# neggles/neurosis

Measured on AMD Instinct MI355X. Metric: train images/sec (node) SDXL 1024^2, higher is better.
Workload: dtype bf16

## Files before the change

### neurosis_amd/csrc/gemm.hip

```cpp
#include "nk_common.h"
#include "nk_gemm.h"
#include <stdlib.h>

#define BM 128
#define BN 128
#define BK 64
#define NTHREADS 256
#define GROUP_M 8
#define KC_IMAGE_BYTES (128 * 128)
#define MC_ROW_BYTES (128 * 2 + 16)
#define MC_IMAGE_BYTES (BK * MC_ROW_BYTES)
#define OPND_BYTES MC_IMAGE_BYTES
#define STAGE_BYTES (2 * OPND_BYTES)
#define CS_LD 132
#define SMEM_BYTES (2 * STAGE_BYTES)

static_assert(SMEM_BYTES >= BM * CS_LD * 4, "epilogue staging must fit");

enum { OP_KC = 0, OP_KCG = 1, OP_MC = 2, OP_MCT = 3, OP_MCG = 4 };

__device__ __forceinline__ bool is_kc(int mode) { return mode == OP_KC || mode == OP_KCG; }

__device__ __forceinline__ long gather_offset(const NkGather& g, int n, int bh, int bw, int kh, int kw,
                                              int c, bool& valid) {
// ... 1097 lines not shown
            int spins = 0;
            bool gave_up = (p.sk_debug & 2) != 0;
            while (!gave_up && __hip_atomic_load(p.sk_flags + ticket, __ATOMIC_RELAXED, __HIP_MEMORY_SCOPE_AGENT) == 0u) {
              __builtin_amdgcn_s_sleep(8);
              if (++spins > (1 << 21)) gave_up = true;
            }
            if (gave_up) {
              if (tid == 0) {
                __hip_atomic_store(p.sk_flags + SK_MAX_GRID + 1, 1u, __ATOMIC_RELAXED, __HIP_MEMORY_SCOPE_AGENT);
                __hip_atomic_store(p.sk_health, 1u, __ATOMIC_RELAXED, __HIP_MEMORY_SCOPE_AGENT);
              }
              const float poison = __builtin_nanf("");
#pragma unroll
              for (int i = 0; i < 4; ++i)
#pragma unroll
                for (int j = 0; j < 2; ++j) acc[i][j] = (float4_t){poison, poison, poison, poison};
              break;
            }
            sk_add_partial(p.sk_ws + (size_t)ticket * SK_TILE_FLOATS, acc, wave, lane);
            __syncthreads();
            if (tid == 0) __hip_atomic_store(p.sk_flags + ticket, 0u, __ATOMIC_RELAXED, __HIP_MEMORY_SCOPE_AGENT);
          }
          if (s_li <= ts) break;
        }
      }
      sk_epilogue<OUT_F32>(p, C, acc, m0, n0, lane, wm, wn);
    }
  }
}

#define XL_BM 256
#define XL_BN 256
#define XL_STAGE_BYTES 65536
#define XL_SMEM_BYTES (2 * XL_STAGE_BYTES)
template <int AMODE, int WM, int WN>
__global__ __launch_bounds__((XL_BM / WM) * (XL_BN / WN) * 64, (XL_BM / WM) * (XL_BN / WN) / 4) void nk_gemm_xl_kernel(const NkGemmParams p) {
  extern __shared__ __attribute__((aligned(16))) char smem[];
  constexpr int WCOLS = XL_BN / WN, NWAVES = (XL_BM / WM) * WCOLS, NP = 32 / NWAVES, MI = WM / 16, NJ = WN / 16;
  const int tid = threadIdx.x, lane = tid & 63, wave = tid >> 6;
  const int wm = wave / WCOLS, wn = wave % WCOLS;
  const int nwg = gridDim.x, bid = blockIdx.x;
  const int q8 = nwg >> 3, r8 = nwg & 7, xcd = bid & 7;
  const int wg = (xcd < r8 ? xcd * (q8 + 1) : r8 * (q8 + 1) + (xcd - r8) * q8) + (bid >> 3);
  const int ntn = (p.N + XL_BN - 1) / XL_BN, ntm = (p.M + XL_BM - 1) / XL_BM;
  constexpr int GM = 4;
  const int per_group = GM * ntn;
  const int group = wg / per_group;
  const int first_m = group * GM;
  const int gm = min(GM, ntm - first_m);
  const int in_group = wg - group * per_group;
  const int nt = in_group / gm;
  const int m0 = (first_m + (in_group - nt * gm)) * XL_BM, n0 = nt * XL_BN;
  const int kend = p.K, nk = (p.K + BK - 1) / BK;

  OperandDMA<AMODE, NP> opa;
  OperandDMA<OP_KC, NP> opb;
  opa.init(p.A, p.lda, p.M, m0, tid, p.ga);
  opb.init(p.B, p.ldb, p.N, n0, tid, p.gb);
  float4_t acc[MI][NJ];
#pragma unroll
  for (int i = 0; i < MI; ++i)
#pragma unroll
    for (int j = 0; j < NJ; ++j) acc[i][j] = (float4_t){0.f, 0.f, 0.f, 0.f};
  opa.start(0);
  opb.start(0);
  if (nk > 0) {
    opa.issue_next(kend, smem, p.ga, p.tw);
    opb.issue_next(kend, smem + 32768, p.gb, p.tw);
  }
  for (int kt = 0; kt < nk; ++kt) {
    asm volatile("s_waitcnt vmcnt(0)" ::: "memory");
    __syncthreads();
    const char* cur = smem + (kt & 1) * XL_STAGE_BYTES;
    if (kt + 1 < nk) {
      char* nxt = smem + ((kt + 1) & 1) * XL_STAGE_BYTES;
      opa.issue_next(kend, nxt, p.ga, p.tw);
      opb.issue_next(kend, nxt + 32768, p.gb, p.tw);
    }
#pragma unroll
    for (int ks = 0; ks < 2; ++ks) {
      bf16x8_t af[MI], bfr[NJ];
#pragma unroll
      for (int i = 0; i < MI; ++i) af[i] = OperandDMA<OP_KC>::frag(cur, wm * WM + i * 16, ks, lane);
#pragma unroll
      for (int j = 0; j < NJ; ++j) bfr[j] = OperandDMA<OP_KC>::frag(cur + 32768, wn * WN + j * 16, ks, lane);
#pragma unroll
      for (int i = 0; i < MI; ++i)
#pragma unroll
        for (int j = 0; j < NJ; ++j)
          acc[i][j] = __builtin_amdgcn_mfma_f32_16x16x32_bf16(bfr[j], af[i], acc[i][j], 0, 0, 0);
    }
  }
#pragma unroll
  for (int ib = 0; ib < MI / 4; ++ib)
#pragma unroll
    for (int half = 0; half < NJ / 2; ++half) {
      float4_t pair[4][2];
#pragma unroll
      for (int i = 0; i < 4; ++i) { pair[i][0] = acc[ib * 4 + i][2 * half]; pair[i][1] = acc[ib * 4 + i][2 * half + 1]; }
      reg_epilogue_64x32<0>(p, p.C, pair, m0 + wm * WM + ib * 64, n0 + wn * WN + half * 32, lane);
    }
}

template <int AMODE, int GEGLU = 0>
__global__ __launch_bounds__(512, 2) void nk_gemm_xl2g_kernel(const NkGemmParams p) {
  extern __shared__ __attribute__((aligned(16))) char smem[];
  const int tid = threadIdx.x, lane = tid & 63, wave = tid >> 6;
  const int wm = wave >> 2, wn = wave & 3;
  const int nwg = gridDim.x, bid = blockIdx.x;
  const int q8 = nwg >> 3, r8 = nwg & 7, xcd = bid & 7;
  const int wg = (xcd < r8 ? xcd * (q8 + 1) : r8 * (q8 + 1) + (xcd - r8) * q8) + (bid >> 3);
  const int ntn = (p.N + XL_BN - 1) / XL_BN, ntm = (p.M + XL_BM - 1) / XL_BM;
  constexpr int GM = 4;
  const int per_group = GM * ntn;
  const int group = wg / per_group;
  const int first_m = group * GM;
  const int gm = min(GM, ntm - first_m);
  const int in_group = wg - group * per_group;
  const int nt = in_group / gm;
  const int m0 = (first_m + (in_group - nt * gm)) * XL_BM, n0 = nt * XL_BN;
  const int kend = p.K, nk = (p.K + BK - 1) / BK;

  OperandDMA<AMODE, 2> a0, a1;
  OperandDMA<OP_KC, 2> b0, b1;
  a0.init(p.A, p.lda, p.M, m0, tid, p.ga);
  a1.init(p.A, p.lda, p.M, m0 + 128, tid, p.ga);
  if constexpr (GEGLU) {
    const int I = p.N >> 1, wv = tid >> 6;
    const int gb0 = wv, gb1 = 8 + wv;
    b0.init(p.B, p.ldb, p.N, ((gb0 & 1) ? I : 0) + (n0 >> 1) + (gb0 >> 1) * 16 - wv * 16, tid, p.gb);
    b1.init(p.B, p.ldb, p.N, ((gb1 & 1) ? I : 0) + (n0 >> 1) + (gb1 >> 1) * 16 - wv * 16, tid, p.gb);
  } else {
    b0.init(p.B, p.ldb, p.N, n0, tid, p.gb);
    b1.init(p.B, p.ldb, p.N, n0 + 128, tid, p.gb);
  }
  const int s0 = p.k_rotate ? (xcd * nk) >> 3 : 0;
  const int wrap_at = nk - s0;
  int na0 = 0, na1 = 0, nb0 = 0, nb1 = 0, ka0 = kend, ka1 = kend, kb0 = kend, kb1 = kend;
  a0.start(s0 * BK); a1.start(s0 * BK); b0.start(s0 * BK); b1.start(s0 * BK);
#define X2_NEXT(op, src, g, cnt, ke)                        \
  do {                                                      \
    op.next_sources(ke, src, g, p.tw);                      \
    if (++cnt == wrap_at) { op.start(0); ke = s0 * BK; }    \
  } while (0)
#define X2_ISSUE(op, img, g, cnt, ke)                       \
  do {                                                      \
    const bf16_t* s_[2];                                    \
    X2_NEXT(op, s_, g, cnt, ke);                            \
    op.fire(0, s_[0], img); op.fire(1, s_[1], img);         \
  } while (0)
  float4_t acc[8][4];
#pragma unroll
  for (int i = 0; i < 8; ++i)
#pragma unroll
    for (int j = 0; j < 4; ++j) acc[i][j] = (float4_t){0.f, 0.f, 0.f, 0.f};

  bf16x8_t ar[8], bc0[4], bc1[4];
  typedef __attribute__((address_space(3))) const char* lds_c;
  const unsigned lds0 = (unsigned)(size_t)(lds_c)smem;
  const unsigned x0 = (unsigned)(((lane >> 4) ^ (lane & 7)) << 4);
  const unsigned arow = lds0 + (unsigned)(wm * 128 + (lane & 15)) * 128u;
  const unsigned brow = lds0 + 32768u + (unsigned)(wn * 64 + (lane & 15)) * 128u;
  const unsigned a_k0 = arow + x0, a_k1 = arow + (x0 ^ 64u), b_k0 = brow + x0, b_k1 = brow + (x0 ^ 64u);
#define X2_RD1(f, addr, OFF) asm volatile("ds_read_b128 %0, %1 offset:%2" : "=v"(f) : "v"(addr), "n"((OFF)))
#define X2_RDA(half)                                                                                             \
  X2_RD1(ar[0], ca0, (half) * 8192); X2_RD1(ar[1], ca0, (half) * 8192 + 2048); X2_RD1(ar[2], ca0, (half) * 8192 + 4096);    \
  X2_RD1(ar[3], ca0, (half) * 8192 + 6144); X2_RD1(ar[4], ca1, (half) * 8192); X2_RD1(ar[5], ca1, (half) * 8192 + 2048);    \
  X2_RD1(ar[6], ca1, (half) * 8192 + 4096); X2_RD1(ar[7], ca1, (half) * 8192 + 6144)
#define X2_RDB(f, half)                                                                                          \
  X2_RD1(f[0], cb0, (half) * 4096); X2_RD1(f[1], cb0, (half) * 4096 + 2048); X2_RD1(f[2], cb1, (half) * 4096);              \
  X2_RD1(f[3], cb1, (half) * 4096 + 2048)
#define X2_BAR() __builtin_amdgcn_sched_barrier(0); __builtin_amdgcn_s_barrier(); __builtin_amdgcn_sched_barrier(0)
#define X2_MM(rb, cb, bf, PREP)                                                                                  \
  asm volatile("s_waitcnt lgkmcnt(0)" ::: "memory");                                                             \
  __builtin_amdgcn_sched_barrier(0);                                                                             \
  __builtin_amdgcn_s_setprio(1);                                                                                 \
  PREP;               \
  _Pragma("unroll") for (int ks = 0; ks < 2; ++ks)                                                               \
    _Pragma("unroll") for (int i = 0; i < 4; ++i)                                                                \
      _Pragma("unroll") for (int j = 0; j < 2; ++j)                                                              \
        acc[(rb) + i][(cb) + j] = __builtin_amdgcn_mfma_f32_16x16x32_bf16(bf[ks * 2 + j], ar[ks * 4 + i], acc[(rb) + i][(cb) + j], 0, 0, 0); \
  __builtin_amdgcn_s_setprio(0)

  const bf16_t* sa0[2];
  const bf16_t* sa1[2];
  const bf16_t* sb0[2];
  const bf16_t* sb1[2];
  if (nk > 0) {
    X2_ISSUE(a0, smem, p.ga, na0, ka0);
    X2_ISSUE(a1, smem + 16384, p.ga, na1, ka1);
    X2_ISSUE(b0, smem + 32768, p.gb, nb0, kb0);
    X2_ISSUE(b1, smem + 49152, p.gb, nb1, kb1);
    X2_ISSUE(b0, smem + XL_STAGE_BYTES + 32768, p.gb, nb0, kb0);
    X2_ISSUE(b1, smem + XL_STAGE_BYTES + 49152, p.gb, nb1, kb1);
    asm volatile("s_waitcnt vmcnt(4)" ::: "memory");
  }
  X2_NEXT(a1, sa1, p.ga, na1, ka1);
  X2_BAR();
  if (wm == 1) { X2_BAR(); }
  for (int t = 0; t < nk; ++t) {
    const unsigned so = (unsigned)(t & 1) * XL_STAGE_BYTES;
    char* cur = smem + so;
    char* oth = smem + (so ^ XL_STAGE_BYTES);
    const unsigned ca0 = a_k0 + so, ca1 = a_k1 + so, cb0 = b_k0 + so, cb1 = b_k1 + so;
    __builtin_amdgcn_sched_barrier(0);
    X2_RDB(bc0, 0);
    X2_RDA(0);
    a1.fire(0, sa1[0], oth + 16384);
    a1.fire(1, sa1[1], oth + 16384);
    X2_BAR();
    X2_MM(0, 0, bc0, X2_NEXT(a0, sa0, p.ga, na0, ka0));
    X2_BAR();
    X2_RDB(bc1, 1);
    a0.fire(0, sa0[0], oth);
    a0.fire(1, sa0[1], oth);
    X2_BAR();
    X2_MM(0, 2, bc1, (void)0);
    X2_BAR();
    X2_RDA(1);
    X2_BAR();
    X2_MM(4, 2, bc1, X2_NEXT(b0, sb0, p.gb, nb0, kb0); X2_NEXT(b1, sb1, p.gb, nb1, kb1));
    X2_BAR();
    b0.fire(0, sb0[0], cur + 32768);
    b0.fire(1, sb0[1], cur + 32768);
    b1.fire(0, sb1[0], cur + 49152);
    b1.fire(1, sb1[1], cur + 49152);
    asm volatile("s_waitcnt vmcnt(4)" ::: "memory");
    X2_BAR();
    X2_MM(4, 0, bc0, X2_NEXT(a1, sa1, p.ga, na1, ka1));
    X2_BAR();
  }
  if (wm == 0) { X2_BAR(); }
  asm volatile("s_waitcnt vmcnt(0)" ::: "memory");
#undef X2_NEXT
#undef X2_ISSUE
#undef X2_RD1
#undef X2_RDA
#undef X2_RDB
#undef X2_BAR
#undef X2_MM
  if constexpr (GEGLU) {
    const int I = p.N >> 1;
    const int abase = (n0 >> 1) + wn * 32;
    const int cl = (lane >> 4) * 4;
    float4_t ba[2], bg[2];
#pragma unroll
    for (int q = 0; q < 2; ++q) {
      ba[q] = p.bias ? *(const float4_t*)(p.bias + abase + q * 16 + cl) : (float4_t){0.f, 0.f, 0.f, 0.f};
      bg[q] = p.bias ? *(const float4_t*)(p.bias + I + abase + q * 16 + cl) : (float4_t){0.f, 0.f, 0.f, 0.f};
    }
    NkGemmParams ph = p;
    ph.N = I; ph.ldc = p.ld_h; ph.bias = nullptr;
    NkGemmParams ps = p;
    ps.bias = nullptr;
#pragma unroll
    for (int ib = 0; ib < 2; ++ib) {
      float4_t pa[4][2], pg[4][2], phh[4][2];
#pragma unroll
      for (int i = 0; i < 4; ++i)
#pragma unroll
        for (int q = 0; q < 2; ++q) {
          pa[i][q] = acc[ib * 4 + i][2 * q];
          pg[i][q] = acc[ib * 4 + i][2 * q + 1];
#pragma unroll
          for (int r = 0; r < 4; ++r) {
            const float av = bf2f(f2bf(pa[i][q][r] + ba[q][r])), gv = bf2f(f2bf(pg[i][q][r] + bg[q][r]));
            float cdf, pdf;
            normal_cdf_pdf(gv, cdf, pdf);
            const float ge = gv * cdf;
            phh[i][q][r] = av * ge;
            if (p.geglu_save) {
              pa[i][q][r] = ge;
              pg[i][q][r] = av * (cdf + gv * pdf);
            }
          }
        }
      const int mb = m0 + wm * 128 + ib * 64;
      if (p.geglu_save) {
        reg_epilogue_64x32<0>(ps, p.C, pa, mb, abase, lane);
        reg_epilogue_64x32<0>(ps, p.C, pg, mb, I + abase, lane);
      } else {
        reg_epilogue_64x32<0>(p, p.C, pa, mb, abase, lane);
        reg_epilogue_64x32<0>(p, p.C, pg, mb, I + abase, lane);
      }
      reg_epilogue_64x32<0>(ph, p.geglu_h, phh, mb, abase, lane);
    }
    return;
  }
#pragma unroll
  for (int ib = 0; ib < 2; ++ib)
#pragma unroll
    for (int half = 0; half < 2; ++half) {
      float4_t pair[4][2];
#pragma unroll
      for (int i = 0; i < 4; ++i) { pair[i][0] = acc[ib * 4 + i][2 * half]; pair[i][1] = acc[ib * 4 + i][2 * half + 1]; }
      reg_epilogue_64x32<0>(p, p.C, pair, m0 + wm * 128 + ib * 64, n0 + wn * 64 + half * 32, lane);
    }
}

static bool use_xl(const NkGemmParams& p, int amode, int bmode, int out_f32, int splitk);
__global__ void nk_zero_f32_kernel(float* __restrict__ dst, size_t n);
#include "gemm_g2.h"
#include "gemm_w160.h"
#include "conv_halo.h"
#include "conv_wgrad_halo.h"

static bool use_xl(const NkGemmParams& p, int amode, int bmode, int out_f32, int splitk) {
  static int on = -1;
  if (on < 0) { const char* e = getenv("NK_GEMM_XL"); on = (e && e[0] == '0') ? 0 : 1; }
  if (!on || p.nbatch || out_f32 || splitk != 1 || bmode != OP_KC || !(amode == OP_KC || amode == OP_KCG)) return false;
  const long ntn = (p.N + XL_BN - 1) / XL_BN;
  const long tiles = (long)((p.M + XL_BM - 1) / XL_BM) * ntn;
  const long rounds = (tiles + 255) / 256;
  return tiles >= 224 && tiles * 10 >= rounds * 256 * 8 && ntn * XL_BN * 100 <= (long)p.N * 112 && p.K >= 4 * BK;
}
template <int AMODE, int WM, int WN>
static int launch_xl_as(const NkGemmParams& p, hipStream_t stream) {
  auto kern = nk_gemm_xl_kernel<AMODE, WM, WN>;
  nk_optin_lds((const void*)kern, XL_SMEM_BYTES);
  dim3 grid(((p.M + XL_BM - 1) / XL_BM) * ((p.N + XL_BN - 1) / XL_BN), 1, 1);
  hipLaunchKernelGGL(kern, grid, dim3((XL_BM / WM) * (XL_BN / WN) * 64), XL_SMEM_BYTES, stream, p);
  return nk_check_launch("nk_gemm_xl_kernel");
}
template <int AMODE>
static int launch_xl(const NkGemmParams& p_in, hipStream_t stream) {
  if (AMODE == OP_KC) {
    auto kern = nk_gemm_xl2g_kernel<OP_KC, 0>;
    auto kerng = nk_gemm_xl2g_kernel<OP_KC, 1>;
    nk_optin_lds((const void*)kern, XL_SMEM_BYTES);
    nk_optin_lds((const void*)kerng, XL_SMEM_BYTES);
    NkGemmParams p = p_in;
    p.k_rotate = k_rotate_on(p.K) ? 1 : 0;
    dim3 grid(((p.M + XL_BM - 1) / XL_BM) * ((p.N + XL_BN - 1) / XL_BN), 1, 1);
    if (p.geglu_h) hipLaunchKernelGGL(kerng, grid, dim3(512), XL_SMEM_BYTES, stream, p);
    else hipLaunchKernelGGL(kern, grid, dim3(512), XL_SMEM_BYTES, stream, p);
    return nk_check_launch("nk_gemm_xl2g_kernel");
  }
  return launch_xl_as<AMODE, 64, 64>(p_in, stream);
}

template <int AMODE, int BMODE, int OUT_F32>
static int launch(const NkGemmParams& p_in, int splitk, hipStream_t stream) {
  NkGemmParams p2 = p_in;
  const NkGemmParams& p = p2;
  auto kern8 = nk_gemm_dma_kernel<AMODE, BMODE, OUT_F32, 8>;
  auto kernr = nk_gemm_ring_kernel<AMODE, BMODE, OUT_F32>;
  nk_optin_lds((const void*)kern8, V2_SMEM_BYTES);
  nk_optin_lds((const void*)kernr, RING_SMEM_BYTES);
  int ntm = (p.M + BM - 1) / BM, ntn = (p.N + BN - 1) / BN;
  dim3 grid(ntm * ntn, splitk, p.nbatch ? p.nbatch : 1);
  {
    int per_xcd = (ntm * ntn + 7) / 8, g = 1;
    while ((g + 1) * (g + 1) <= per_xcd) ++g;
    p2.group_m = g > GROUP_M ? GROUP_M : g;
  }
  p2.k_rotate = k_rotate_on(splitk > 1 ? p.ksplit_len : p.K) ? 1 : 0;
  if (!p.nbatch && (long)ntm * ntn * splitk <= 256) {
    hipLaunchKernelGGL(kernr, grid, dim3(512), RING_SMEM_BYTES, stream, p);
    return nk_check_launch("nk_gemm_ring_kernel");
  }
  hipLaunchKernelGGL(kern8, grid, dim3(512), V2_SMEM_BYTES, stream, p);
  return nk_check_launch("nk_gemm_dma_kernel");
}


#include <mutex>
#include <unordered_map>
struct SkWorkspace {
  unsigned* counter = nullptr;
  unsigned* flags = nullptr;
  float* ws = nullptr;
};
static std::mutex sk_mutex;
static std::unordered_map<void*, SkWorkspace> sk_spaces;

static bool use_sk(const NkGemmParams& p, int out_f32) {
  int mode = 4;
  if (const char* e = getenv("NK_GEMM_SK")) mode = atoi(e);
  if (mode == 0) return false;
  if (mode == 1) return true;
  if (mode == 2) return out_f32 != 0;
  if (mode == 4 && out_f32) return false;
  const long tiles = (long)((p.M + BM - 1) / BM) * ((p.N + BN - 1) / BN) * (p.nbatch ? p.nbatch : 1);
  const long nk = (p.K + BK - 1) / BK;
  const long rounds = (tiles + 511) / 512;
  const double fill = (double)tiles / (double)(rounds * 512);
  if (tiles >= 1024 && fill >= 0.8) return false;
  if (tiles >= 512 && fill >= 0.95) return false;
  return nk >= 24;
}

static int sk_prepare(NkGemmParams& p, int grid, hipStream_t stream) {
  std::lock_guard<std::mutex> lock(sk_mutex);
  SkWorkspace& w = sk_spaces[(void*)stream];
  if (!w.ws) {
    hipStreamCaptureStatus capturing = hipStreamCaptureStatusNone;
    if (hipStreamIsCapturing(stream, &capturing) == hipSuccess && capturing != hipStreamCaptureStatusNone) {
      nk_set_error(__FILE__, __LINE__, "stream-K workspace requested while the stream is capturing: run the launch once on this stream before capturing it");
      return NK_ERR_LAUNCH;
    }
    char* raw = nullptr;
    const size_t ws_bytes = (size_t)SK_MAX_GRID * SK_TILE_FLOATS * sizeof(float);
    if (hipMalloc((void**)&raw, ws_bytes + (SK_MAX_GRID + 64) * sizeof(unsigned)) != hipSuccess) {
      nk_set_error(__FILE__, __LINE__, "hipMalloc of the stream-K workspace failed");
      return NK_ERR_LAUNCH;
    }
    w.ws = (float*)raw;
    w.flags = (unsigned*)(raw + ws_bytes);
    w.counter = w.flags + SK_MAX_GRID;
    if (hipMemsetAsync(w.flags, 0, (SK_MAX_GRID + 64) * sizeof(unsigned), stream) != hipSuccess) return NK_ERR_LAUNCH;
  }
  p.sk_health = nk_health_word();
  if (!p.sk_health) { nk_set_error(__FILE__, __LINE__, "health word allocation failed"); return NK_ERR_LAUNCH; }
  p.sk_counter = w.counter;
  p.sk_flags = w.flags;
  p.sk_ws = w.ws;
  p.sk_base = 0;
  p.sk_epoch = 0;
  return NK_OK;
}

int nk_gemm_sk_reset(void) {
  std::lock_guard<std::mutex> lock(sk_mutex);
  for (auto& kv : sk_spaces)
    if (kv.second.flags && hipMemset(kv.second.flags, 0, (SK_MAX_GRID + 64) * sizeof(unsigned)) != hipSuccess) return NK_ERR_LAUNCH;
  return NK_OK;
}

extern "C" int nk_gemm_sk_status(void) {
  std::lock_guard<std::mutex> lock(sk_mutex);
  if (hipDeviceSynchronize() != hipSuccess) return -1;
  int bad = 0;
  for (auto& kv : sk_spaces) {
    unsigned v = 0;
    if (kv.second.flags && hipMemcpy(&v, kv.second.flags + SK_MAX_GRID + 1, sizeof(v), hipMemcpyDeviceToHost) == hipSuccess && v) bad = 1;
  }
  return bad;
}

template <int AMODE, int BMODE, int OUT_F32>
static int launch_sk(NkGemmParams& p, hipStream_t stream) {
  auto kern = nk_gemm_sk_kernel<AMODE, BMODE, OUT_F32>;
  nk_optin_lds((const void*)kern, SK_SMEM_BYTES);
  const long ntm = (p.M + BM - 1) / BM, ntn = (p.N + BN - 1) / BN, nk = (p.K + BK - 1) / BK;
  const long T = ntm * ntn * (p.nbatch ? p.nbatch : 1), W = T * nk;
  const int max_grid = SK_MAX_GRID & ~7, min_iters = 4;
  long grid = (W / min_iters) & ~7l;
  if (grid > max_grid) grid = max_grid;
  if (grid < 8) grid = 8;
  p.sk_chunked = T >= 64;
  { const char* d = getenv("NK_SK_DEBUG"); p.sk_debug = d ? atoi(d) & 2 : 0; }
  if (int e = sk_prepare(p, (int)grid, stream)) return e;
  hipLaunchKernelGGL(kern, dim3((unsigned)grid), dim3(SK_NT), SK_SMEM_BYTES, stream, p);
  return nk_check_launch("nk_gemm_sk_kernel");
}

__global__ __launch_bounds__(256) void nk_zero_f32_kernel(float* __restrict__ dst, size_t n) {
  const size_t n4 = n / 4, stride = (size_t)gridDim.x * 256;
  float4_t* d4 = (float4_t*)dst;
  for (size_t i = (size_t)blockIdx.x * 256 + threadIdx.x; i < n4; i += stride) d4[i] = (float4_t){0.f, 0.f, 0.f, 0.f};
  if (blockIdx.x == 0 && threadIdx.x < (n & 3)) dst[n4 * 4 + threadIdx.x] = 0.f;
}

static int pick_splitk(int M, int N, int K, int max_split) {
  int tiles = ((M + BM - 1) / BM) * ((N + BN - 1) / BN);
  int nk = (K + BK - 1) / BK;
  const int lo = 96, hi = 192;
  if (tiles >= lo && tiles * 2 <= 512 && nk >= 256 && max_split >= 2) return 2;
  if (tiles >= lo) return 1;
  int s = 1;
  while (s < max_split && tiles * s < hi && nk / (s * 2) >= 8) s *= 2;
  return s;
}

static void set_split(NkGemmParams& p, int splitk) {
  int nk = (p.K + BK - 1) / BK;
  int per = (nk + splitk - 1) / splitk;
  p.ksplit_len = per * BK;
}

static int zero_split_outputs(const NkGemmParams& p, hipStream_t stream) {
  for (int z = 0; z < (p.nbatch ? p.nbatch : 1); ++z) {
    const size_t n = (size_t)p.M * p.N;
    float* dst = (float*)(p.nbatch ? p.Cb[z] : p.C);
    const unsigned blocks = (unsigned)((n / 4 + 255) / 256 > 2048 ? 2048 : (n / 4 + 255) / 256);
    hipLaunchKernelGGL(nk_zero_f32_kernel, dim3(blocks ? blocks : 1), dim3(256), 0, stream, dst, n);
    float* db = p.nbatch ? p.dbias_b[z] : p.dbias;
    if (db) hipLaunchKernelGGL(nk_zero_f32_kernel, dim3(1), dim3(256), 0, stream, db, (size_t)p.M);
  }
  return hipGetLastError() != hipSuccess ? NK_ERR_LAUNCH : NK_OK;
}

int nk_gemm_dispatch(NkGemmParams& p, int amode, int bmode, int out_f32, int allow_splitk,
                     hipStream_t stream) {
  NK_CHECK_ARG(p.M > 0 && p.N > 0 && p.K > 0);
  if (!p.nbatch) NK_CHECK_ARG(((uintptr_t)p.A & 15) == 0 && ((uintptr_t)p.B & 15) == 0 && ((uintptr_t)p.C & 15) == 0);
  for (int z = 0; z < p.nbatch; ++z) NK_CHECK_ARG(((uintptr_t)p.Ab[z] & 15) == 0 && ((uintptr_t)p.Bb[z] & 15) == 0 && ((uintptr_t)p.Cb[z] & 15) == 0);
  if (amode == OP_KC) NK_CHECK_ARG((p.K & 7) == 0 && (p.lda & 7) == 0);
  if (bmode == OP_KC) NK_CHECK_ARG((p.K & 7) == 0 && (p.ldb & 7) == 0);
  if (amode == OP_KCG) NK_CHECK_ARG((p.ga.C & 7) == 0);
  if (amode == OP_MC) NK_CHECK_ARG((p.M & 7) == 0 && (p.lda & 7) == 0);
  if (bmode == OP_MC) NK_CHECK_ARG((p.N & 7) == 0 && (p.ldb & 7) == 0);
  if (bmode == OP_MCT) NK_CHECK_ARG((p.N & 7) == 0 && (p.tw.co_stride & 7) == 0 && (p.tw.tap_stride & 7) == 0);
  if (bmode == OP_MCG) NK_CHECK_ARG((p.gb.C & 7) == 0);
  if (p.residual) NK_CHECK_ARG(((uintptr_t)p.residual & 15) == 0 && ((p.ldr & 7) == 0 || (p.N & 7) != 0));
  if (!out_f32) NK_CHECK_ARG((p.ldc & 7) == 0 || (p.N & 7) != 0);
  if (p.fRowsPerBatch.d == 0) p.fRowsPerBatch = make_fastdiv(1);

  if (p.dbias || (p.nbatch && p.dbias_b[0])) NK_CHECK_ARG(amode == OP_MC && out_f32);
  if (p.geglu_h) {
    NK_CHECK_ARG(amode == OP_KC && bmode == OP_KC && !out_f32 && !p.nbatch && (p.N & 255) == 0 && (p.ld_h & 7) == 0 && !p.rowvec && !p.residual && p.alpha == 1.0f);
    NK_CHECK_ARG(((uintptr_t)p.geglu_h & 15) == 0 && (!p.bias || ((uintptr_t)p.bias & 15) == 0));
    if (!use_xl(p, amode, bmode, out_f32, 1)) {
      nk_set_error(__FILE__, __LINE__, "fused GEGLU forward on a shape the 256 x 256 kernel does not take (ask nk_linear_fwd_geglu_ok first)");
      return NK_ERR_ARG;
    }
    set_split(p, 1);
    return launch_xl<OP_KC>(p, stream);
  }
  if (p.geglu_u) {
    NK_CHECK_ARG(amode == OP_KC && bmode == OP_MC && !out_f32 && !p.nbatch && (p.N & 7) == 0 && (p.ld_u & 7) == 0 && !p.bias && !p.rowvec && !p.residual);
    set_split(p, 1);
    return launch<OP_KC, OP_MC, 0>(p, 1, stream);
  }
  if (use_halo(p, amode, bmode, out_f32)) return launch_halo(p, stream);
  if (use_wgrad_halo(p, amode, bmode, out_f32)) return launch_wgrad_halo(p, stream);
  if (p.stats_part) {
    nk_set_error(__FILE__, __LINE__, "statistics epilogue on a convolution the halo-tile kernel does not take (ask nk_conv2d_stats_tiles first)");
    return NK_ERR_ARG;
  }

  {
    const W160Plan wp = w160_plan(p, amode, bmode, out_f32, allow_splitk);
    if (wp.bn) {
      set_split(p, wp.splitk);
      if (wp.splitk > 1 && p.accumulate == 0) {
        NK_CHECK_ARG(p.ldc == p.N);
        if (int rc = zero_split_outputs(p, stream)) return rc;
        p.accumulate = 1;
      } else if (p.accumulate == 2) {
        p.accumulate = wp.splitk > 1 ? 1 : 0;
      }
      p.k_rotate = k_rotate_on(wp.splitk > 1 ? p.ksplit_len : p.K) ? 1 : 0;
      return wp.bn == 160 ? launch_w160_as<160>(p, wp.splitk, stream) : launch_w160_as<128>(p, wp.splitk, stream);
    }
  }
  if (use_ring64(p, amode, bmode, out_f32)) return launch_ring64(p, stream);
  if ((!p.nbatch || p.nbatch <= NK_MAX_BATCH) && use_g2(p, amode, bmode, out_f32, 1) && (g2_mode() == 2 || !use_xl(p, amode, bmode, out_f32, 1))) {
    if (p.accumulate == 2) p.accumulate = 0;
    if (amode == OP_KC && bmode == OP_KC) return out_f32 ? launch_g2<OP_KC, OP_KC, 1>(p, stream) : launch_g2<OP_KC, OP_KC, 0>(p, stream);
    if (amode == OP_KC && bmode == OP_MC) return out_f32 ? launch_g2<OP_KC, OP_MC, 1>(p, stream) : launch_g2<OP_KC, OP_MC, 0>(p, stream);
    if (amode == OP_KCG && bmode == OP_KC) return out_f32 ? launch_g2<OP_KCG, OP_KC, 1>(p, stream) : launch_g2<OP_KCG, OP_KC, 0>(p, stream);
    if (amode == OP_KCG && bmode == OP_MCT) return out_f32 ? launch_g2<OP_KCG, OP_MCT, 1>(p, stream) : launch_g2<OP_KCG, OP_MCT, 0>(p, stream);
    return out_f32 ? launch_g2<OP_MC, OP_MC, 1>(p, stream) : launch_g2<OP_MC, OP_MC, 0>(p, stream);
  }

  bool has_dbias = p.dbias != nullptr;
  for (int z = 0; z < p.nbatch && z < NK_MAX_BATCH; ++z) has_dbias = has_dbias || p.dbias_b[z] != nullptr;
  if (!has_dbias && use_sk(p, out_f32)) {
    const long ntm_ = (p.M + BM - 1) / BM, ntn_ = (p.N + BN - 1) / BN, nk_ = (p.K + BK - 1) / BK;
    if (ntm_ * ntn_ * (p.nbatch ? p.nbatch : 1) * nk_ < (1l << 22)) {
      if (p.accumulate == 2) p.accumulate = 0;
#define NK_SK_CASE(A_, B_)                                                        \
      if (amode == A_ && bmode == B_) return out_f32 ? launch_sk<A_, B_, 1>(p, stream) : launch_sk<A_, B_, 0>(p, stream);
      NK_SK_CASE(OP_KC, OP_KC)
      NK_SK_CASE(OP_KC, OP_MC)
      NK_SK_CASE(OP_MC, OP_MC)
      NK_SK_CASE(OP_KCG, OP_KC)
      NK_SK_CASE(OP_KCG, OP_MCT)
      NK_SK_CASE(OP_MC, OP_MCG)
#undef NK_SK_CASE
    }
  }
  int splitk = 1;
  if (out_f32 && allow_splitk) splitk = pick_splitk(p.M * (p.nbatch ? p.nbatch : 1), p.N, p.K, 32);
  if (p.nbatch) NK_CHECK_ARG(p.nbatch <= NK_MAX_BATCH);
  set_split(p, splitk);
  if (out_f32 && splitk > 1 && p.accumulate == 0) {
    NK_CHECK_ARG(p.ldc == p.N);
    if (int rc = zero_split_outputs(p, stream)) return rc;
    p.accumulate = 1;
  } else if (p.accumulate == 2) {
    p.accumulate = splitk > 1 ? 1 : 0;
  }

  if (use_xl(p, amode, bmode, out_f32, splitk))
    return amode == OP_KC ? launch_xl<OP_KC>(p, stream) : launch_xl<OP_KCG>(p, stream);

#define NK_CASE(A_, B_)                                                          \
  if (amode == A_ && bmode == B_) {                                              \
    return out_f32 ? launch<A_, B_, 1>(p, splitk, stream) : launch<A_, B_, 0>(p, splitk, stream); \
  }
  NK_CASE(OP_KC, OP_KC)
  NK_CASE(OP_KC, OP_MC)
  NK_CASE(OP_MC, OP_MC)
  NK_CASE(OP_KCG, OP_KC)
  NK_CASE(OP_KCG, OP_MCT)
  NK_CASE(OP_MC, OP_MCG)
#undef NK_CASE
  nk_set_error(__FILE__, __LINE__, "unsupported operand mode combination");
  return NK_ERR_ARG;
}

int nk_halo_bn(int N) { return halo_bn(N); }
int nk_halo_tiles_per_image(const NkGemmParams& p) {
  if (!use_halo(p, OP_KCG, OP_KC, 0)) return 0;
  return halo_tiles_per_image(p);
}


int nk_geglu_fwd_fusable(const NkGemmParams& p) {
  return (p.N & 255) == 0 && use_xl(p, OP_KC, OP_KC, 0, 1) ? 1 : 0;
}
```

Baseline: 25.88.

## Add persistent warp-specialized GEGLU forward GEMM kernel with triple-buffered loads

Result: faster. 26.32, median of 6 (+1.7%).

```diff
diff --git a/neurosis_amd/csrc/gemm.hip b/neurosis_amd/csrc/gemm.hip
--- a/neurosis_amd/csrc/gemm.hip
+++ b/neurosis_amd/csrc/gemm.hip
@@ -1423,6 +1423,7 @@
 __global__ void nk_zero_f32_kernel(float* __restrict__ dst, size_t n);
 #include "gemm_g2.h"
 #include "gemm_w160.h"
+#include "gemm_geglu_persist.h"
 #include "conv_halo.h"
 #include "conv_wgrad_halo.h"
 
@@ -1637,6 +1638,7 @@
       return NK_ERR_ARG;
     }
     set_split(p, 1);
+    if (use_geglu_persist(p)) return launch_geglu_persist(p, stream);
     return launch_xl<OP_KC>(p, stream);
   }
   if (p.geglu_u) {
diff --git a/neurosis_amd/csrc/gemm_geglu_persist.h b/neurosis_amd/csrc/gemm_geglu_persist.h
--- /dev/null
+++ b/neurosis_amd/csrc/gemm_geglu_persist.h
@@ -0,0 +1,314 @@
+#pragma once
+
+#define GP_BM 256
+#define GP_BN 128
+#define GP_NS 3
+#define GP_A_BYTES (GP_BM * 128)
+#define GP_B_BYTES (GP_BN * 128)
+#define GP_STAGE (GP_A_BYTES + GP_B_BYTES)
+#define GP_BIAS_OFF (GP_NS * GP_STAGE)
+#define GP_SMEM (GP_BIAS_OFF + 2 * 1024)
+#define GP_PPS 12
+
+#define GP_ST_TILES 16
+#define GP_ST_WORDS (4 + 3 * GP_ST_TILES)
+#ifdef NK_GEGLU_STAMPS
+__device__ unsigned long long nk_geglu_stamp_buf[GP_ST_WORDS * 1024];
+#define GP_STAMP(slot) do { if (wave == 0 && lane == 0 && blockIdx.x < 1024) nk_geglu_stamp_buf[blockIdx.x * GP_ST_WORDS + (slot)] = __builtin_amdgcn_s_memtime(); } while (0)
+#define GP_PSTAMP_DECL unsigned long long ps_fire = 0, ps_wait = 0, ps_bar = 0, ps_t = 0
+#define GP_PSTAMP_T() (ps_t = __builtin_amdgcn_s_memtime())
+#define GP_PSTAMP_ADD(acc) do { const unsigned long long n_ = __builtin_amdgcn_s_memtime(); acc += n_ - ps_t; ps_t = n_; } while (0)
+#define GP_PSTAMP_OUT() do { if (wave == 4 && lane == 0 && blockIdx.x < 1024) { nk_geglu_stamp_buf[blockIdx.x * GP_ST_WORDS + 1] = ps_fire; nk_geglu_stamp_buf[blockIdx.x * GP_ST_WORDS + 2] = ps_wait; nk_geglu_stamp_buf[blockIdx.x * GP_ST_WORDS + 3] = ps_bar; } } while (0)
+#else
+#define GP_STAMP(slot)
+#define GP_PSTAMP_DECL
+#define GP_PSTAMP_T()
+#define GP_PSTAMP_ADD(acc)
+#define GP_PSTAMP_OUT()
+#endif
+
+__device__ __forceinline__ void gp_tile(int T, int ntiles, int ntm, int ntn, int& m0, int& ac0) {
+  const int q8 = ntiles >> 3, r8 = ntiles & 7, xcd = T & 7;
+  const int wg = (xcd < r8 ? xcd * (q8 + 1) : r8 * (q8 + 1) + (xcd - r8) * q8) + (T >> 3);
+  constexpr int GM = 4;
+  const int per_group = GM * ntn;
+  const int group = wg / per_group;
+  const int first_m = group * GM;
+  const int gm = min(GM, ntm - first_m);
+  const int in_group = wg - group * per_group;
+  const int nt = in_group / gm;
+  m0 = (first_m + (in_group - nt * gm)) * GP_BM;
+  ac0 = nt * (GP_BN / 2);
+}
+
+template <typename F, int... G>
+__device__ __forceinline__ void gp_unroll(F&& f, std::integer_sequence<int, G...>) { (f(std::integral_constant<int, G>{}), ...); }
+
+template <int MI>
+__device__ __forceinline__ void gp_store_x32(bf16_t* C, long ldc, const float4_t (&v)[MI][2], int mbase, int nbase, int lane) {
+  const int g = lane >> 4;
+  const int n = nbase + (g & 1) * 16 + (g >> 1) * 8;
+  const int mrow = mbase + (lane & 15);
+#pragma unroll
+  for (int i = 0; i < MI; ++i) {
+    uint4_t o;
+    auto lo = __builtin_amdgcn_permlane16_swap(pack2bf(v[i][0][0], v[i][0][1]), pack2bf(v[i][1][0], v[i][1][1]), false, false);
+    auto hi = __builtin_amdgcn_permlane16_swap(pack2bf(v[i][0][2], v[i][0][3]), pack2bf(v[i][1][2], v[i][1][3]), false, false);
+    o.x = lo[0]; o.y = hi[0]; o.z = lo[1]; o.w = hi[1];
+    *(uint4_t*)(C + (long)(mrow + i * 16) * ldc + n) = o;
+  }
+}
+
+#define GP_RD(f, addr, OFF) asm volatile("ds_read_b128 %0, %1 offset:%2" : "=v"(f) : "v"(addr), "n"((OFF)))
+#define GP_BAR() __builtin_amdgcn_sched_barrier(0); __builtin_amdgcn_s_barrier(); __builtin_amdgcn_sched_barrier(0)
+
+template <int SAVE>
+__global__ __launch_bounds__(512, 1) void nk_gemm_geglu_persist_kernel(const NkGemmParams p) {
+  extern __shared__ __attribute__((aligned(16))) char smem[];
+  const int wave = __builtin_amdgcn_readfirstlane(threadIdx.x >> 6);
+  const int I = p.N >> 1;
+  const int ntm = (p.M + GP_BM - 1) / GP_BM, ntn = I / (GP_BN / 2), ntiles = ntm * ntn;
+  const int grid = gridDim.x, bid = blockIdx.x;
+  const int my_tiles = bid < ntiles ? (ntiles - bid + grid - 1) / grid : 0;
+  const int nk = p.K / BK;
+
+  if (wave >= 4) {
+    const int pw = wave - 4;
+    const int lane = (int)__builtin_amdgcn_mbcnt_hi(~0u, __builtin_amdgcn_mbcnt_lo(~0u, 0u));
+    const bf16_t* const zp = (const bf16_t*)nk_zero_page;
+    const int krow = lane >> 3, kchunk = (lane & 7) ^ (lane >> 3);
+    const bf16_t* base[GP_PPS];
+    bool live[GP_PPS];
+    const bf16_t* bsrc = zp;
+    const int s0 = p.k_rotate ? ((bid & 7) * nk) >> 3 : 0;
+    int ct = 0, t = 0, kslab = 0;
+    auto load_tile = [&](int T) {
+      int m0, ac0;
+      gp_tile(T, ntiles, ntm, ntn, m0, ac0);
+#pragma unroll
+      for (int i = 0; i < GP_PPS; ++i) {
+        const int pc = pw + 4 * i;
+        if (i < 8) {
+          const int r = m0 + pc * 8 + krow;
+          live[i] = r < p.M;
+          base[i] = live[i] ? p.A + (long)r * p.lda + kchunk * 8 : zp;
+        } else {
+          const int br = (pc - 32) * 8 + krow, gb = br >> 4;
+          const int wr = ((gb & 1) ? I : 0) + ac0 + (gb >> 1) * 16 + (br & 15);
+          live[i] = true;
+          base[i] = p.B + (long)wr * p.ldb + kchunk * 8;
+        }
+      }
+      if (pw == 0) {
+        const int c = lane < 16 ? ac0 + 4 * lane : I + ac0 + 4 * (lane - 16);
+        bsrc = (p.bias && lane < 32) ? (const bf16_t*)(p.bias + c) : zp;
+      }
+    };
+    auto fire_next = [&](char* stage) -> bool {
+      if (ct >= my_tiles) {
+#pragma unroll
+        for (int i = 0; i < GP_PPS; ++i) __builtin_amdgcn_global_load_lds((nk_gptr)zp, (nk_lptr)(stage + (pw + 4 * i) * 1024), 16, 0, 0);
+        return false;
+      }
+      if (t == 0) { load_tile(bid + ct * grid); kslab = s0; }
+      const int koff = kslab * BK;
+#pragma unroll
+      for (int i = 0; i < GP_PPS; ++i)
+        __builtin_amdgcn_global_load_lds((nk_gptr)(live[i] ? base[i] + koff : zp), (nk_lptr)(stage + (pw + 4 * i) * 1024), 16, 0, 0);
+      const bool bias = pw == 0 && t == 0;
+      if (bias) __builtin_amdgcn_global_load_lds((nk_gptr)bsrc, (nk_lptr)(smem + GP_BIAS_OFF + (ct & 1) * 1024), 16, 0, 0);
+      if (++kslab == nk) kslab = 0;
+      if (++t == nk) { t = 0; ++ct; }
+      return bias;
+    };
+    fire_next(smem);
+    fire_next(smem + GP_STAGE);
+    asm volatile("s_waitcnt vmcnt(%0)" ::"n"(GP_PPS) : "memory");
+    GP_BAR();
+    const int S = my_tiles * nk;
+    unsigned sn = 2 * GP_STAGE;
+    GP_PSTAMP_DECL;
+    GP_PSTAMP_T();
+    for (int g = 0; g < S; ++g) {
+      const bool bias = fire_next(smem + sn);
+      GP_PSTAMP_ADD(ps_fire);
+      if (bias) asm volatile("s_waitcnt vmcnt(%0)" ::"n"(GP_PPS + 1) : "memory");
+      else asm volatile("s_waitcnt vmcnt(%0)" ::"n"(GP_PPS) : "memory");
+      GP_PSTAMP_ADD(ps_wait);
+      GP_BAR();
+      GP_PSTAMP_ADD(ps_bar);
+      sn += GP_STAGE; if (sn == GP_NS * GP_STAGE) sn = 0;
+    }
+    GP_PSTAMP_OUT();
+    asm volatile("s_waitcnt vmcnt(0)" ::: "memory");
+    return;
+  }
+
+  const int lane = (int)__builtin_amdgcn_mbcnt_hi(~0u, __builtin_amdgcn_mbcnt_lo(~0u, 0u));
+  __builtin_amdgcn_s_setprio(1);
+  typedef __attribute__((address_space(3))) const char* lds_c;
+  const unsigned lds0 = (unsigned)(size_t)(lds_c)smem;
+  const unsigned x0 = (unsigned)(((lane >> 4) ^ (lane & 7)) << 4);
+  const unsigned arow = lds0 + (unsigned)(wave * 64 + (lane & 15)) * 128u;
+  const unsigned brow = lds0 + (unsigned)GP_A_BYTES + (unsigned)(lane & 15) * 128u;
+  unsigned ra[2] = {arow + x0, arow + (x0 ^ 64u)}, rb[2] = {brow + x0, brow + (x0 ^ 64u)};
+  auto set_stage = [&](unsigned delta) {
+    ra[0] += delta; ra[1] += delta; rb[0] += delta; rb[1] += delta;
+  };
+  bf16x8_t af[2][4], bf[2][8];
+  float4_t acc[4][8];
+  auto issue_read = [&](auto p_tag, auto ks_tag, auto r_tag) {
+    constexpr int P = decltype(p_tag)::value, KS = decltype(ks_tag)::value, R = decltype(r_tag)::value;
+    auto& A_ = af[P];
+    auto& B_ = bf[P];
+    const unsigned a_ = ra[KS], b_ = rb[KS];
+    if constexpr (R < 8) GP_RD(B_[R], b_, R * 2048);
+    else GP_RD(A_[R - 8], a_, (R - 8) * 2048);
+  };
+  auto wait_all = [&](auto p_tag) {
+    constexpr int P = decltype(p_tag)::value;
+    asm volatile("s_waitcnt lgkmcnt(0)" : "+v"(bf[P][0]), "+v"(bf[P][1]), "+v"(bf[P][2]), "+v"(bf[P][3]), "+v"(bf[P][4]), "+v"(bf[P][5]),
+                 "+v"(bf[P][6]), "+v"(bf[P][7]), "+v"(af[P][0]), "+v"(af[P][1]), "+v"(af[P][2]), "+v"(af[P][3]));
+    __builtin_amdgcn_sched_barrier(0);
+  };
+  auto substep = [&](auto cur_tag, auto nks_tag, auto barrier_tag, auto reads_tag, unsigned so_delta) {
+    constexpr int CUR = decltype(cur_tag)::value, NKS = decltype(nks_tag)::value;
+    constexpr bool BARRIER = decltype(barrier_tag)::value, READS = decltype(reads_tag)::value;
+    constexpr int NXT = 1 - CUR, G0 = BARRIER ? 8 : 0;
+    auto gap = [&acc, &af, &bf, &set_stage, &issue_read, so_delta](auto g_tag) {
+      constexpr int g = decltype(g_tag)::value, i = g >> 3, j = g & 7;
+      acc[i][j] = __builtin_amdgcn_mfma_f32_16x16x32_bf16(bf[CUR][j], af[CUR][i], acc[i][j], 0, 0, 0);
+      if constexpr (BARRIER && g == 7) {
+        GP_BAR();
+        set_stage(so_delta);
+      }
+      if constexpr (READS && g >= G0 && g < G0 + 12) issue_read(std::integral_constant<int, NXT>{}, std::integral_constant<int, NKS>{}, std::integral_constant<int, g - G0>{});
+      __builtin_amdgcn_sched_barrier(0);
+    };
+    gp_unroll(gap, std::make_integer_sequence<int, 32>{});
+    if constexpr (READS) wait_all(std::integral_constant<int, NXT>{});
+  };
+  auto first_reads = [&]() {
+    gp_unroll([&](auto r_tag) { issue_read(std::integral_constant<int, 0>{}, std::integral_constant<int, 0>{}, r_tag); }, std::make_integer_sequence<int, 12>{});
+    wait_all(std::integral_constant<int, 0>{});
+  };
+
+  GP_BAR();
+  first_reads();
+
+  const int cl = (lane >> 4) * 4;
+  unsigned so = 0;
+  for (int ct = 0; ct < my_tiles; ++ct) {
+#pragma unroll
+    for (int i = 0; i < 4; ++i)
+#pragma unroll
+      for (int j = 0; j < 8; ++j) acc[i][j] = (float4_t){0.f, 0.f, 0.f, 0.f};
+#ifdef NK_GEGLU_STAMPS
+    if (ct < GP_ST_TILES) GP_STAMP(4 + 3 * ct);
+#endif
+    auto next_stage = [](unsigned o) { o += GP_STAGE; return o == GP_NS * GP_STAGE ? 0u : o; };
+    for (int t = 0; t + 1 < nk; ++t) {
+      const unsigned son = next_stage(so);
+      substep(std::integral_constant<int, 0>{}, std::integral_constant<int, 1>{}, std::false_type{}, std::true_type{}, 0u);
+      substep(std::integral_constant<int, 1>{}, std::integral_constant<int, 0>{}, std::true_type{}, std::true_type{}, son - so);
+      so = son;
+    }
+    {
+      const unsigned son = next_stage(so);
+      substep(std::integral_constant<int, 0>{}, std::integral_constant<int, 1>{}, std::false_type{}, std::true_type{}, 0u);
+      substep(std::integral_constant<int, 1>{}, std::integral_constant<int, 0>{}, std::true_type{}, std::false_type{}, son - so);
+      so = son;
+    }
+#ifdef NK_GEGLU_STAMPS
+    if (ct < GP_ST_TILES) GP_STAMP(5 + 3 * ct);
+#endif
+    int m0, ac0;
+    gp_tile(bid + ct * grid, ntiles, ntm, ntn, m0, ac0);
+    const float* bl = (const float*)(smem + GP_BIAS_OFF + (ct & 1) * 1024);
+    const int mb = m0 + wave * 64;
+#pragma unroll
+    for (int h = 0; h < 2; ++h) {
+      float4_t ba[2], bg[2];
+#pragma unroll
+      for (int q = 0; q < 2; ++q) {
+        ba[q] = *(const float4_t*)(bl + (2 * h + q) * 16 + cl);
+        bg[q] = *(const float4_t*)(bl + 64 + (2 * h + q) * 16 + cl);
+      }
+#pragma unroll
+      for (int ih = 0; ih < 4; ++ih) {
+        float4_t pa[1][2], pg[1][2], phh[1][2];
+#pragma unroll
+        for (int q = 0; q < 2; ++q) {
+          const int qq = 2 * h + q;
+#pragma unroll
+          for (int i = 0; i < 1; ++i) {
+#pragma unroll
+            for (int r = 0; r < 4; ++r) {
+              const float ua = acc[ih + i][2 * qq][r] + ba[q][r], ug = acc[ih + i][2 * qq + 1][r] + bg[q][r];
+              const unsigned ag = pack2bf(ua, ug);
+              const float av = __uint_as_float(ag << 16), gv = __uint_as_float(ag & 0xffff0000u);
+              float cdf, pdf;
+              normal_cdf_pdf(gv, cdf, pdf);
+              const float ge = gv * cdf;
+              phh[i][q][r] = av * ge;
+              if constexpr (SAVE) {
+                pa[i][q][r] = ge;
+                pg[i][q][r] = av * (cdf + gv * pdf);
+              } else {
+                pa[i][q][r] = ua;
+                pg[i][q][r] = ug;
+              }
+            }
+          }
+        }
+        const int ab = ac0 + h * 32, m = mb + ih * 16;
+        gp_store_x32<1>((bf16_t*)p.C, p.ldc, pa, m, ab, lane);
+        gp_store_x32<1>((bf16_t*)p.C, p.ldc, pg, m, I + ab, lane);
+        gp_store_x32<1>(p.geglu_h, p.ld_h, phh, m, ab, lane);
+        __builtin_amdgcn_sched_barrier(0);
+      }
+    }
+#ifdef NK_GEGLU_STAMPS
+    if (ct < GP_ST_TILES) GP_STAMP(6 + 3 * ct);
+#endif
+    first_reads();
+  }
+  __builtin_amdgcn_s_setprio(0);
+}
+#undef GP_RD
+#undef GP_BAR
+#ifdef NK_GEGLU_STAMPS
+extern "C" int nk_debug_geglu_stamps(unsigned long long* host_out, int nwg) {
+  return hipMemcpyFromSymbol(host_out, HIP_SYMBOL(nk_geglu_stamp_buf), (size_t)nwg * GP_ST_WORDS * sizeof(unsigned long long)) == hipSuccess ? 0 : 1;
+}
+#endif
+
+static int gp_cu_count() {
+  static int cached[16] = {0};
+  int dev = 0;
+  (void)hipGetDevice(&dev);
+  if (dev < 0 || dev >= 16) dev = 0;
+  if (!cached[dev]) {
+    int n = 0;
+    if (hipDeviceGetAttribute(&n, hipDeviceAttributeMultiprocessorCount, dev) != hipSuccess || n <= 0) n = 256;
+    cached[dev] = n;
+  }
+  return cached[dev];
+}
+static bool use_geglu_persist(const NkGemmParams& p) {
+  const char* e = getenv("NK_GEGLU_PERSIST");
+  if (e && atoi(e) == 0) return false;
+  if (p.M % GP_BM || (p.N >> 1) % (GP_BN / 2) || p.K % BK || p.K / BK < 4) return false;
+  const long tiles = (long)(p.M / GP_BM) * ((p.N >> 1) / (GP_BN / 2));
+  return tiles % gp_cu_count() == 0;
+}
+static int launch_geglu_persist(const NkGemmParams& p_in, hipStream_t stream) {
+  NkGemmParams p = p_in;
+  p.k_rotate = k_rotate_on(p.K) ? 1 : 0;
+  auto kern = p.geglu_save ? nk_gemm_geglu_persist_kernel<1> : nk_gemm_geglu_persist_kernel<0>;
+  nk_optin_lds((const void*)kern, GP_SMEM);
+  const long tiles = (long)(p.M / GP_BM) * ((p.N >> 1) / (GP_BN / 2));
+  const int grid = (int)std::min<long>(tiles, gp_cu_count());
+  hipLaunchKernelGGL(kern, dim3(grid), dim3(512), GP_SMEM, stream, p);
+  return nk_check_launch("nk_gemm_geglu_persist_kernel");
+}
```
